# Ulixes-8/UNet-Implementations

Measured on AMD Instinct MI355X. Metric: images/sec (512x512, bs/GPU=8) Our_UNet train step, higher is better.
Workload: dtype f32; 1 GPU; Our_UNet 6-stage 3-class 512x512 bs=8/GPU fp32 train step (fwd + Dice/wCE loss + bwd + SGD-Nesterov), train mode, HIP conv/IN/upsample kernels; global_batch=8, parallelism=dp1, world=1

## Files before the change

include/unet_hip.h:

```cpp
#ifndef UNET_HIP_H_
#define UNET_HIP_H_

#include <stddef.h>
#include <stdint.h>

#ifdef __cplusplus
extern "C" {
#endif

#define UNET_ABI_VERSION 11

#define UNET_OK 0
#define UNET_E_INVALID (-1)
#define UNET_E_LAUNCH (-2)
#define UNET_E_WORKSPACE (-3)

typedef void* unet_stream_t;

const char* unet_last_error(void);
int unet_abi_version(void);
int unet_device_count(void);

int unet_debug_set_chunk_limit(int64_t bytes);

// ... 179 lines not shown
int unet_augment_u8(const uint8_t* image, const uint8_t* mask, uint8_t* image_out,
                    uint8_t* mask_out, const float* params, const uint32_t* rng, int N, int H,
                    int W, unet_stream_t stream);

int unet_preprocess_u8(const uint8_t* image_hwc, const uint8_t* mask, float* out_nhwc,
                       int64_t* target, int N, int H, int W, const float* mean3, const float* std3,
                       unet_stream_t stream);


int unet_sgd_nesterov_step(float* params, const float* grads, float* momentum, int64_t n,
                           float lr, float mu, float weight_decay, int first_step,
                           float grad_scale, unet_stream_t stream);

int unet_sgd_nesterov_step_dev(float* params, const float* grads, float* momentum, int64_t n,
                               const float* hyper, int first_step, unet_stream_t stream);

typedef struct unet_act_src {
  const float* x;
  int C;
  const float* alpha;
  const float* beta;
} unet_act_src;

size_t unet_conv_in_fwd_workspace_bytes(int N, int H, int W, int Cout, int stride);
int unet_conv_in_fwd(const unet_act_src* s0, const unet_act_src* s1, float slope, const float* w,
                     const float* bias, int ksize, int stride, float* y, void* workspace,
                     size_t workspace_bytes, int* stats_px_out, int N, int H, int W, int Cout,
                     unet_stream_t stream);
int unet_conv_in_fwd_bf16x3(const unet_act_src* s0, const unet_act_src* s1, float slope,
                            const float* w, const uint16_t* w3, const float* bias, int ksize,
// ... 292 lines not shown
```

unet-implementations_amd/_lib.py:

```python
import ctypes
import os
import subprocess

_HERE = os.path.dirname(os.path.abspath(__file__))
LIB_PATH = os.environ.get("UNET_HIP_LIB") or os.path.join(_HERE, "libunet_hip.so")
CSRC = os.path.join(_HERE, "csrc")

ABI_VERSION = 11

_c = ctypes
_p = _c.c_void_p
_i = _c.c_int
_f = _c.c_float
_sz = _c.c_size_t
_i64 = _c.c_int64



class ActSrc(ctypes.Structure):
    _fields_ = [("x", _p), ("C", _i), ("alpha", _p), ("beta", _p)]


_ps = _c.POINTER(ActSrc)

# ... 56 lines not shown
    "unet_wgrad_defer_flush": (_i, [_p]),
    "unet_wgrad_defer_end": (_i, [_p]),
    "unet_dice_wce_loss_grad": (_i, [_p, _p, _p, _sz, _p, _p, _i, _i, _i, _i, _p]),
    "unet_argmax_dice_counts": (_i, [_p, _p, _p, _p, _i, _i, _i, _i, _p]),
    "unet_eval_confusion": (_i, [_p, _p, _p, _p, _i, _i, _i, _i, _p]),
    "unet_eval_maps": (_i, [_p, _p, _p, _p, _p, _i, _i, _i, _p]),
    "unet_augment_params_per_sample": (_i, []),
    "unet_augment_u8": (_i, [_p, _p, _p, _p, _p, _p, _i, _i, _i, _p]),
    "unet_gradcam_workspace_bytes": (_sz, [_i, _i, _i]),
    "unet_gradcam_weights": (_i, [_p, _i, _p, _p, _sz, _i, _i, _i, _p]),
    "unet_gradcam_map": (_i, [_ps, _i, _f, _p, _p, _p, _sz, _i, _i, _p]),
    "unet_gradcam_heatmap": (_i, [_p, _p, _sz, _p, _i, _i, _i, _i, _i, _p]),
    "unet_preprocess_u8": (_i, [_p, _p, _p, _p, _i, _i, _i, _c.POINTER(_f), _c.POINTER(_f), _p]),
    "unet_sgd_nesterov_step": (_i, [_p, _p, _p, _i64, _f, _f, _f, _i, _f, _p]),
    "unet_sgd_nesterov_step_dev": (_i, [_p, _p, _p, _i64, _p, _i, _p]),
    "unet_conv_in_fwd_workspace_bytes": (_sz, [_i, _i, _i, _i, _i]),
    "unet_conv_in_fwd": (_i, [_ps, _ps, _f, _p, _p, _i, _i, _p, _p, _sz, _c.POINTER(_i), _i, _i, _i,
                              _i, _p]),
    "unet_conv_in_fwd_bf16x3": (_i, [_ps, _ps, _f, _p, _p, _p, _i, _i, _p, _p, _sz, _c.POINTER(_i), _i,
                                     _i, _i, _i, _p]),
    "unet_conv_up_in_fwd_supported": (_i, [_i, _i, _i, _i, _i, _i]),
    "unet_conv_up_in_fwd": (_i, [_ps, _ps, _f, _p, _p, _p, _p, _sz, _c.POINTER(_i), _i, _i, _i, _i,
                                 _p]),
    "unet_conv_in_stats_finalize": (_i, [_p, _p, _sz, _i, _p, _p, _f, _p, _p, _p, _p, _p, _i, _i, _i,
                                         _p]),
    "unet_stem_u8_fwd": (_i, [_p, _c.POINTER(_f), _c.POINTER(_f), _p, _p, _p, _p, _sz,
                              _c.POINTER(_i), _i, _i, _i, _i, _p]),
    "unet_stem_u8_bwd_weight": (_i, [_p, _c.POINTER(_f), _c.POINTER(_f), _p, _p, _p, _sz, _i, _i,
                                     _i, _i, _p]),
    "unet_conv_in_bwd_weight": (_i, [_ps, _f, _p, _p, _i, _i, _i, _i, _p, _sz, _i, _i, _i, _i, _p]),
# ... 144 lines not shown
```

unet-implementations_amd/csrc/conv_wino.hip:

```cpp
#include "conv_params.h"
#include "lds_asm.h"
#include <utility>

namespace unet_conv {
namespace {

typedef int i32x4v __attribute__((ext_vector_type(4)));
template <int I> using wn_ic = std::integral_constant<int, I>;
template <int B, int... I, typename F>
__device__ __forceinline__ void wn_for_impl(std::integer_sequence<int, I...>, F&& f) {
  (f(wn_ic<B + I>{}), ...);
}
template <int B, int E, typename F>
__device__ __forceinline__ void wn_for(F&& f) {
  wn_for_impl<B>(std::make_integer_sequence<int, E - B>{}, f);
}

constexpr int WN_TH = 8, WN_TW = 32;
constexpr int WN_PW = WN_TW + 2, WN_PH = WN_TH + 2;
constexpr int WN_PPIX = WN_PH * WN_PW;
constexpr int WN_BN = 64;
constexpr int WN_KC = 8;
constexpr int WN_RP = 360;
constexpr int WN_BUF = 16 * 64 * WN_KC;
constexpr size_t WN_LDS = (size_t)(4 * WN_BUF + 2 * WN_KC * WN_RP) * sizeof(float);

__host__ __device__ __forceinline__ int wn_swz(int row, int k) {
  return 2 * ((k >> 1) ^ ((row >> 2) & 3)) + (k & 1);
}

struct WinoParams {
  IgemmParams g;
  const float* wu;
};

template <bool ACT, bool STATS, bool BSTATS, bool UP = false>
__global__ __launch_bounds__(512, 2) void conv_wino_kernel(const WinoParams wp) {
  const IgemmParams& p = wp.g;
  extern __shared__ __attribute__((aligned(16))) float smem[];
// ... 403 lines not shown

__device__ __forceinline__ void wino_pack_items(const float* __restrict__ w,
                                                float* __restrict__ uf, float* __restrict__ ud,
                                                int Cout, int Cin, int dir, long long block) {
  float* dst = dir == 0 ? uf : ud;
  if (!dst) return;
  const int Nn = dir == 0 ? Cout : Cin, Kt = dir == 0 ? Cin : Cout;
  const int kchunks = Kt / WN_KC;
  const long long items = (long long)Nn * kchunks;
  const long long idx = block * 256 + threadIdx.x;
  if (idx >= items) return;
  const int nl = (int)(idx & 63);
  const long long rest = idx >> 6;
  const int kc = (int)(rest % kchunks), tn = (int)(rest / kchunks);
  const int nn = tn * WN_BN + nl;
  float u[16][8];
#pragma unroll
  for (int k = 0; k < 8; ++k) {
    const int kk = kc * WN_KC + k;
    const int co = dir == 0 ? nn : kk, ci = dir == 0 ? kk : nn;
    const float* g = w + ((size_t)co * Cin + ci) * 9;
    float t4[4][3];
#pragma unroll
    for (int v = 0; v < 3; ++v) {
      const float g0 = dir == 0 ? g[0 + v] : g[6 + 2 - v];
      const float g1 = dir == 0 ? g[3 + v] : g[3 + 2 - v];
      const float g2 = dir == 0 ? g[6 + v] : g[0 + 2 - v];
      t4[0][v] = g0;
      t4[1][v] = 0.5f * (g0 + g1 + g2);
      t4[2][v] = 0.5f * (g0 - g1 + g2);
      t4[3][v] = g2;
    }
#pragma unroll
    for (int a = 0; a < 4; ++a) {
      u[4 * a + 0][k] = t4[a][0];
      u[4 * a + 1][k] = 0.5f * (t4[a][0] + t4[a][1] + t4[a][2]);
      u[4 * a + 2][k] = 0.5f * (t4[a][0] - t4[a][1] + t4[a][2]);
      u[4 * a + 3][k] = t4[a][2];
    }
  }
  const bool s1 = (nl >> 2) & 1, s2 = (nl >> 3) & 1;
  float* blk = dst + ((size_t)tn * kchunks + kc) * WN_BUF + nl * 8;
#pragma unroll
  for (int x = 0; x < 16; ++x) {
    f32x2v p0 = {u[x][0], u[x][1]}, p1 = {u[x][2], u[x][3]}, p2 = {u[x][4], u[x][5]},
           p3 = {u[x][6], u[x][7]};
    const f32x2v q0 = s1 ? p1 : p0, q1 = s1 ? p0 : p1, q2 = s1 ? p3 : p2, q3 = s1 ? p2 : p3;
    p0 = s2 ? q2 : q0; p1 = s2 ? q3 : q1; p2 = s2 ? q0 : q2; p3 = s2 ? q1 : q3;
    *reinterpret_cast<f32x4*>(blk + x * 512) = f32x4{p0[0], p0[1], p1[0], p1[1]};
    *reinterpret_cast<f32x4*>(blk + x * 512 + 4) = f32x4{p2[0], p2[1], p3[0], p3[1]};
  }
}

__global__ __launch_bounds__(256) void wino_pack_kernel(const float* __restrict__ w,
                                                        float* __restrict__ uf,
                                                        float* __restrict__ ud, int Cout, int Cin) {
  wino_pack_items(w, uf, ud, Cout, Cin, blockIdx.y, blockIdx.x);
}
__global__ __launch_bounds__(256) void wino_pack_batched_kernel(
    const unet_wino_pack_entry* __restrict__ tab, int n) {
  int k = 0;
  for (int q = 1; q < n; ++q)
    if (tab[q].block_begin <= (int)blockIdx.x) k = q;
  const unet_wino_pack_entry e = tab[k];
  wino_pack_items(e.w, e.uf, e.ud, e.Cout, e.Cin, blockIdx.y, (long long)blockIdx.x - e.block_begin);
}
// ... 153 lines not shown
```

unet-implementations_amd/csrc/misc.hip:

```cpp
#include "conv_params.h"

#include <cxxabi.h>
#include <stdlib.h>
#include <string.h>

#include <mutex>
#include <string>
#include <vector>

static thread_local char g_err[512] = "";

void unet_set_error(const char* fmt, ...) {
  va_list ap;
  va_start(ap, fmt);
  vsnprintf(g_err, sizeof(g_err), fmt, ap);
  va_end(ap);
}

extern "C" const char* unet_last_error(void) { return g_err; }

namespace unet_conv {
long long& chunk_limit_bytes() {
  static long long lim = (1LL << 31) - 1;
  return lim;
// ... 513 lines not shown
    float acc = 0.f;
    for (int Y = ylo; Y <= yhi; ++Y) {
      const float cy = bil_coef(Y, sy, h, iy);
      if (cy == 0.f) continue;
      float row = 0.f;
      for (int X = xlo; X <= xhi; ++X) {
        const float cx = bil_coef(X, sx, w, ix);
        if (cx != 0.f) row += cx * g[(size_t)Y * W + X];
      }
      acc += cy * row;
    }
    gx[i] = acc;
  }
}

__global__ __launch_bounds__(256) void sgd_nesterov_kernel(float* __restrict__ p,
                                                           const float* __restrict__ g,
                                                           float* __restrict__ buf, long long n,
                                                           float lr, float mu, float wd,
                                                           int first_step, float gscale,
                                                           const float* __restrict__ hyper) {
  if (hyper) { lr = hyper[0]; mu = hyper[1]; wd = hyper[2]; gscale = hyper[3]; }
  const long long stride = (long long)gridDim.x * 256;
  const long long n4 = n >> 2;
  for (long long i = (long long)blockIdx.x * 256 + threadIdx.x; i < n4; i += stride) {
    f32x4 pv = *reinterpret_cast<f32x4*>(p + i * 4);
    f32x4 gv = *reinterpret_cast<const f32x4*>(g + i * 4) * gscale + pv * wd;
    f32x4 bv;
    if (first_step) bv = gv;
    else bv = *reinterpret_cast<f32x4*>(buf + i * 4) * mu + gv;
    *reinterpret_cast<f32x4*>(buf + i * 4) = bv;
    gv += bv * mu;
    pv -= gv * lr;
    *reinterpret_cast<f32x4*>(p + i * 4) = pv;
  }
  if (blockIdx.x == 0 && threadIdx.x < (n & 3)) {
    const long long i = (n4 << 2) + threadIdx.x;
    float pv = p[i];
    float gv = g[i] * gscale + pv * wd;
    float bv = first_step ? gv : buf[i] * mu + gv;
    buf[i] = bv;
    gv += bv * mu;
    p[i] = pv - gv * lr;
  }
}

unsigned stream_grid(long long items) {
  long long b = ceil_div64(items, 256);
  if (b > 256 * 16) b = 256 * 16;
  if (b < 1) b = 1;
  return (unsigned)b;
}

}

extern "C" int unet_nchw_to_nhwc(const float* x, float* y, int N, int C, int H, int W,
                                 unet_stream_t stream) {
  UNET_REQUIRE(x && y && N > 0 && C > 0 && H > 0 && W > 0, "nchw_to_nhwc: bad argument");
// ... 149 lines not shown

extern "C" int unet_sgd_nesterov_step_dev(float* params, const float* grads, float* momentum,
                                          int64_t n, const float* hyper, int first_step,
                                          unet_stream_t stream) {
  UNET_REQUIRE(params && grads && momentum && hyper && n > 0, "sgd_nesterov_step_dev: bad argument");
  UNET_REQUIRE(((uintptr_t)params % 16 == 0) && ((uintptr_t)grads % 16 == 0) &&
                   ((uintptr_t)momentum % 16 == 0),
               "sgd_nesterov_step_dev: arenas must be 16-byte aligned");
  hipLaunchKernelGGL(sgd_nesterov_kernel, dim3(stream_grid((n + 3) / 4)), dim3(256), 0,
                     (hipStream_t)stream, params, grads, momentum, (long long)n, 0.f, 0.f, 0.f,
                     first_step, 1.f, hyper);
  UNET_CHECK_LAUNCH("sgd_nesterov(dev)");
  return UNET_OK;
}

extern "C" int unet_transpose2d(const float* src, float* dst, int R, int C, unet_stream_t stream) {
  UNET_REQUIRE(src && dst && R > 0 && C > 0, "transpose2d: bad argument");
  hipLaunchKernelGGL(transpose2d_kernel, dim3(ceil_div(C, 32), ceil_div(R, 32)), dim3(256), 0,
                     (hipStream_t)stream, src, dst, R, C);
  UNET_CHECK_LAUNCH("transpose2d");
  return UNET_OK;
}

extern "C" int unet_preprocess_u8(const uint8_t* image_hwc, const uint8_t* mask, float* out_nhwc,
                                  int64_t* target, int N, int H, int W, const float* mean3,
                                  const float* std3, unet_stream_t stream) {
  UNET_REQUIRE(image_hwc && out_nhwc && mean3 && std3 && N > 0 && H > 0 && W > 0 &&
                   (mask == nullptr || target != nullptr),
               "preprocess_u8: bad argument");
  const long long pixels = (long long)N * H * W;
// ... 30 lines not shown
```

unet-implementations_amd/ddp.py:

```python
import torch
import torch.distributed as dist


class GradBucketAllReduce:

    def __init__(self, model, optimizer=None, process_group=None, bucket_bytes=16 << 20,
                 average=True, always_reduce=False):
        if not dist.is_initialized():
            raise RuntimeError("torch.distributed must be initialised (backend nccl or gloo)")
        self.model = model
        self.group = process_group
        self.world = dist.get_world_size(process_group)
        self.bucket_elems = max(1, bucket_bytes // 4)
        self._works = []
        self._hi = None
        self._prefix = 0
        self.sent_ranges = []
        self.always_reduce = always_reduce
        model.grad_ready_hook = self._on_ready
        if optimizer is not None:
            optimizer.grad_scale = 1.0 / self.world if average else 1.0

    def _on_ready(self, lo):
        garena = getattr(self.model, "_grad_arena", None)
# ... 41 lines not shown

    def finish(self):
        self.check_gradients_alias_arena()
        if self._hi is not None and self._hi > 0 and (self.world > 1 or self.always_reduce):
            _, garena = self.model.flat_parameters()
            self._launch(garena, self._prefix, self._hi)
        for w in self._works:
            w.wait()
        self._works = []
        self._hi = None


def broadcast_parameters(model, src=0, process_group=None):
    arena, _ = model.flat_parameters()
    dist.broadcast(arena, src=src, group=process_group)
```

unet-implementations_amd/ops.py:

```python
import ctypes
import functools
import struct
import threading

import torch

from ._lib import ActSrc, BwdStats, check, lib


_raw_stream = getattr(torch._C, "_cuda_getCurrentRawStream", None)
_raw_device = getattr(torch._C, "_cuda_getDevice", None)


def _stream():
    if _raw_stream is not None and _raw_device is not None:
        return _raw_stream(_raw_device())
    return torch.cuda.current_stream().cuda_stream


class KernelTimer:

    def __init__(self, only=None):
        self.only = only
        self.records = []
# ... 182 lines not shown
        wd = _f32((9, Cin, Cout), w_oihw)
    check(lib().unet_pack_conv3x3_weights(_ptr(w_oihw), _ptr(wf), _ptr(wd), Cout, Cin, _stream()))
    return wf, wd


def pack_conv3x3_weights_bf16x3(w_oihw, want_wd=True, want_wf=True):
    Cout, Cin, kh, kw = w_oihw.shape
    assert kh == 3 and kw == 3
    wf3 = torch.empty((3, 9, Cout, Cin), dtype=torch.bfloat16, device=w_oihw.device) \
        if want_wf else None
    wd3 = torch.empty((3, 9, Cin, Cout), dtype=torch.bfloat16, device=w_oihw.device) \
        if want_wd else None
    check(lib().unet_pack_conv3x3_weights_bf16x3(_ptr(w_oihw), _ptr(wf3), _ptr(wd3), Cout, Cin,
                                                 _stream()))
    return wf3, wd3


class PackTable:

    def __init__(self, weights, planes, wino=None):
        self.wf, self.wd, self.wf3, self.wd3 = [], [], [], []
        self.src_ptrs = [w.data_ptr() for w in weights]
        self.planes = planes
        self.wino = tuple(wino) if wino is not None else tuple((False, False) for _ in weights)
        self.uf, self.ud, self._wino_jobs = [], [], []
        for w, (ff, fd) in zip(weights, self.wino):
            cout, cin = w.shape[0], w.shape[1]
            uf = _f32((16 * cout * cin,), w) if ff else None
            ud = _f32((16 * cout * cin,), w) if fd else None
            self.uf.append(uf)
# ... 19 lines not shown
            wf = _f32((9, cout, cin), w)
            wd = _f32((9, cin, cout), w)
            wf3 = wd3 = None
            if planes and cin != 3:
                npl = 1 if planes == 1 and planes is not True else 3
                wf3 = torch.empty((npl, 9, cout, cin), dtype=torch.bfloat16, device=w.device)
                wd3 = torch.empty((npl, 9, cin, cout), dtype=torch.bfloat16, device=w.device)
            self.wf.append(wf); self.wd.append(wd); self.wf3.append(wf3); self.wd3.append(wd3)
            raw += struct.pack("<5Q4i", w.data_ptr(), wf.data_ptr(), wd.data_ptr(),
                               0 if wf3 is None else wf3.data_ptr(),
                               0 if wd3 is None else wd3.data_ptr(), cout, cin, tiles,
                               1 if (wf3 is not None and wf3.shape[0] == 1) else 0)
            tiles += (cout // 32) * ((cin + 31) // 32)
        self.n, self.tiles = len(weights), tiles
        self.table = torch.frombuffer(bytearray(raw), dtype=torch.uint8).to(weights[0].device)

    def matches(self, weights, planes, wino=None):
        wino = tuple(wino) if wino is not None else tuple((False, False) for _ in weights)
        return planes == self.planes and len(weights) == self.n and wino == self.wino and \
            all(w.data_ptr() == p for w, p in zip(weights, self.src_ptrs))

    def run(self):
        check(lib().unet_pack_conv3x3_weights_batched(self.table.data_ptr(), self.n, self.tiles,
                                                      _stream()))
        if self._wino_table is not None:
            check(lib().unet_pack_wino_weights_batched(self._wino_table.data_ptr(),
                                                       len(self._wino_jobs), self._wino_blocks,
                                                       _stream()))


_PREC = {False: 0, True: 1, 0: 0, 1: 1, 3: 3, "fp32": 0, "bf16": 1, "bf16x3": 3}
_SUFFIX = {0: "", 1: "_bf16", 3: "_bf16x3"}


def _prec(bf16):
    try:
        return _PREC[bf16]
    except (KeyError, TypeError):
        raise ValueError("precision must be 'fp32', 'bf16' or 'bf16x3'") from None


@functools.lru_cache(maxsize=None)
def _sel_conv3x3_fwd(pr, C0):
# ... 897 lines not shown
    n = params.numel()
    t0 = _begin()
    check(lib().unet_sgd_nesterov_step(_ptr(params), _ptr(grads), _ptr(momentum), n, lr, mu,
                                       weight_decay, 1 if first_step else 0, grad_scale,
                                       _stream()))
    if t0 is not None:
        _timer.end("sgd_nesterov", 0.0, 1, t0, nbytes=4.0 * (5 if not first_step else 4) * n)


def sgd_nesterov_step_dev(params, grads, momentum, hyper, first_step):
    n = params.numel()
    check(lib().unet_sgd_nesterov_step_dev(_ptr(params), _ptr(grads), _ptr(momentum), n,
                                           _ptr(hyper), 1 if first_step else 0, _stream()))


def recon3x3_fwd(x, slope, w, b):
    x, rx = _act(x)
    N, H, W, C = x.shape
    K = w.shape[0]
    out = _f32((N, K, H, W), x.x)
    t0 = _begin()
    check(lib().unet_recon3x3_fwd(rx, 1 if _is_b16(x.x) else 0, slope, _ptr(w), _ptr(b),
                                  _ptr(out), N, H, W, K, _stream()))
    if t0 is not None:
        _timer.end("recon_fwd", 2.0 * N * H * W * K * C * 9, 1, t0,
                   nbytes=x.x.element_size() * x.x.numel() + 4.0 * out.numel())
    return out


_recon_ws = {}
# ... 218 lines not shown
```

unet-implementations_amd/optim.py:

```python
import torch

from . import ops


class FusedSGD(torch.optim.Optimizer):
    def __init__(self, params, lr=1e-3, momentum=0.0, dampening=0.0, weight_decay=0.0,
                 nesterov=False, model=None):
        if dampening != 0.0:
            raise NotImplementedError("FusedSGD implements dampening == 0 (the reference setting)")
        if nesterov and momentum <= 0:
            raise ValueError("Nesterov momentum requires a momentum")
        if not nesterov:
            raise NotImplementedError("FusedSGD implements the Nesterov form used by the reference")
        defaults = dict(lr=lr, momentum=momentum, dampening=dampening, weight_decay=weight_decay,
                        nesterov=nesterov)
        super().__init__(params, defaults)
        self._model = model
        self._flat_buf = None
        self._steps = 0
        self.grad_scale = 1.0
        self._hyper = None
        self._hyper_host = None

    def use_device_hyper(self, on=True):
# ... 53 lines not shown
                self._flat_buf[off:off + p.numel()].view_as(p).copy_(st["momentum_buffer"])
                fresh = False
            st["momentum_buffer"] = self._flat_buf[off:off + p.numel()].view_as(p)
        return fresh

    def _snapshot(self):
        self.adopt_flat_momentum()
        return self._flat_buf.detach().clone(), self._steps

    def _restore(self, snap):
        self._flat_buf.copy_(snap[0])
        self._steps = snap[1]

    def _advanced(self):
        self._steps += 1

    @torch.no_grad()
    def step(self, closure=None):
        loss = None
        if closure is not None:
            with torch.enable_grad():
                loss = closure()
        flat = self._flat_ready()
        if not flat and self.grad_scale != 1.0 and self._model is not None:
            m = self._model
            _, garena = m.flat_parameters()
            for (name, p), off in zip(m.named_parameters(), m._offsets):
                if p.grad is not None and p.grad.data_ptr() != garena.data_ptr() + 4 * off:
                    raise RuntimeError(f"{name}.grad does not alias the gradient arena the "
                                       "all-reduce operates on")
        if flat:
            g = self.param_groups[0]
            arena, garena = self._model.flat_parameters()
            first = bool(self.adopt_flat_momentum())
            if self._hyper is not None:
                self.sync_device_hyper()
                ops.sgd_nesterov_step_dev(arena, garena, self._flat_buf, self._hyper, first)
            else:
                ops.sgd_nesterov_step(arena, garena, self._flat_buf, g["lr"], g["momentum"],
                                      g["weight_decay"], first, self.grad_scale)
        else:
            if self._hyper is not None:
                raise RuntimeError("device-side hyper-parameters need the flat-arena step (every "
                                   "parameter and gradient a view of the UNet arenas)")
            for g in self.param_groups:
                for p in g["params"]:
                    if p.grad is None:
                        continue
                    st = self.state[p]
                    first = "momentum_buffer" not in st or st["momentum_buffer"] is None
                    if first:
                        st["momentum_buffer"] = torch.zeros_like(p)
                    if p.data_ptr() % 16 or p.grad.data_ptr() % 16 or not p.is_contiguous() \
                            or not p.grad.is_contiguous():
                        raise RuntimeError("FusedSGD needs contiguous, 16-byte aligned tensors")
                    ops.sgd_nesterov_step(p.data.view(-1), p.grad.view(-1),
# ... 129 lines not shown
    @torch.no_grad()
    def step(self, closure=None):
        loss = None
        if closure is not None:
            with torch.enable_grad():
                loss = closure()
        flat = self._flat_ready()
        if not flat and self.grad_scale != 1.0 and self._model is not None:
            m = self._model
            _, garena = m.flat_parameters()
            for (name, p), off in zip(m.named_parameters(), m._offsets):
                if p.grad is not None and p.grad.data_ptr() != garena.data_ptr() + 4 * off:
                    raise RuntimeError(f"{name}.grad does not alias the gradient arena the "
                                       "all-reduce operates on")
        self.sync_device_hyper()
        if flat:
            arena, garena = self._model.flat_parameters()
            self.adopt_flat_moments()
            ops.adam_step(arena, garena, self._flat_m, self._flat_v, self._hyper, True)
        else:
            first = True
            for p in self.param_groups[0]["params"]:
                if p.grad is None:
                    continue
                if p.grad.is_sparse:
                    raise RuntimeError("FusedAdam does not support sparse gradients")
                st = self.state[p]
                if st.get("exp_avg") is None:
                    st["exp_avg"] = torch.zeros_like(p, memory_format=torch.preserve_format)
                    st["exp_avg_sq"] = torch.zeros_like(p, memory_format=torch.preserve_format)
# ... 11 lines not shown
```

unet-implementations_amd/train.py:

```python
import torch

from . import ops
from .losses import SimpleLoss
from .optim import FusedAdam, FusedSGD
from .unet import UNet


def create_model(device="cuda"):
    model = UNet(in_channels=3, num_classes=3, n_stages=6,
                 features_per_stage=[32, 64, 128, 256, 512, 512], kernel_sizes=[[3, 3]] * 6,
                 strides=[[1, 1], [2, 2], [2, 2], [2, 2], [2, 2], [2, 2]],
                 n_conv_per_stage=[2] * 6, n_conv_per_stage_decoder=[2] * 5, conv_bias=True,
                 norm_op=torch.nn.InstanceNorm2d, norm_op_kwargs={"eps": 1e-5, "affine": True},
                 dropout_op=None, nonlin=torch.nn.LeakyReLU, nonlin_kwargs={"inplace": True},
                 encoder_dropout_rates=[0.0, 0.0, 0.1, 0.2, 0.3, 0.3],
                 decoder_dropout_rates=[0.3, 0.2, 0.2, 0.1, 0.0])
    return model.to(device)


def create_optimizer(model, lr=0.005, weight_decay=1e-4, momentum=0.99):
    return FusedSGD(model.parameters(), lr=lr, weight_decay=weight_decay, momentum=momentum,
                    nesterov=True, model=model)


# ... 52 lines not shown
        with torch.cuda.stream(side):
            for _ in range(max(1, warmup)):
                train_step(model, optimizer, loss_function, self.images, self.masks,
                           grad_sync=finish, input_layout=input_layout)
        cur.wait_stream(side)
        self.graph = torch.cuda.CUDAGraph()
        mode = "thread_local" if grad_sync is not None else "global"
        if grad_sync is not None:
            torch.cuda.synchronize()
        with torch.cuda.graph(self.graph, capture_error_mode=mode):
            self.loss = train_step(model, optimizer, loss_function, self.images, self.masks,
                                   grad_sync=finish, input_layout=input_layout)
        with torch.no_grad():
            arena.copy_(keep_arena)
            optimizer._restore(keep_opt)

    def __call__(self, images, masks):
        if images.shape != self.images.shape or masks.shape != self.masks.shape:
            raise ValueError("GraphedTrainStep was captured for batches of shape "
                             f"{tuple(self.images.shape)} / {tuple(self.masks.shape)}")
        if images.dtype != self.images.dtype or masks.dtype != self.masks.dtype:
            raise ValueError("GraphedTrainStep was captured for batches of dtype "
                             f"{self.images.dtype} / {self.masks.dtype}")
        if images.data_ptr() != self.images.data_ptr():
            self.images.copy_(images, non_blocking=True)
        if masks.data_ptr() != self.masks.data_ptr():
            self.masks.copy_(masks, non_blocking=True)
        self.optimizer.sync_device_hyper()
        self.graph.replay()
        self.optimizer._advanced()
        return self.loss


@torch.no_grad()
def validate(model, val_loader, loss_function, device, ignore_label=255, input_layout=None):
    model.eval()
    val_loss = torch.zeros((), device=device)
    dice_sum = torch.zeros(3, device=device, dtype=torch.float64)
    n = 0
    for batch in val_loader:
        images = batch["image"].to(device, non_blocking=True)
        masks = batch["mask"].to(device, non_blocking=True)
        outputs = model(images) if input_layout is None else \
            model(images, input_layout=input_layout)
# ... 91 lines not shown
```

unet-implementations_amd/unet.py:

```python
from typing import Dict, List, Optional, Tuple, Type, Union

import torch
import torch.nn as nn

from . import ops


class SpatialDropout2d(nn.Module):

    def __init__(self, drop_prob):
        super().__init__()
        self.drop_prob = drop_prob

    def extra_repr(self):
        return f"drop_prob={self.drop_prob}"

    def draw_mask(self, n, channels, device):
        mask = torch.empty(n, channels, 1, 1, device=device).bernoulli_(1 - self.drop_prob)
        return mask.div_(1 - self.drop_prob).view(n, channels)

    def forward(self, x):
        if not self.training or self.drop_prob == 0:
            return x
        return x * self.draw_mask(x.size(0), x.size(1), x.device).view(x.size(0), x.size(1), 1, 1)
# ... 266 lines not shown
                        n_convs=n_conv_per_stage_decoder[lvl],
                        spatial_dropout_rate=decoder_dropout_rates[s], **common))
        self._build_head(features_per_stage[0], num_classes)
        self.initialize_weights()
        self._plan = None
        self._arena = None
        self._grad_arena = None
        self._offsets = None
        self.dropout_mask_override = None
        self.grad_ready_hook = None
        self.matmul_precision = "fp32"
        self.fused_pipeline = True
        self.winograd = True
        self.fullres_folds = True
        self.wgrad32_folds = True
        self.input_mean, self.input_std = ops.IMAGENET_MEAN, ops.IMAGENET_STD

    def _build_bottleneck(self, common):
        """Hook for variants that add modules between encoder and decoder (CLIPUNet)."""

    def _build_head(self, in_features, out_channels):
        self.segmentation_output = nn.Conv2d(in_features, out_channels, kernel_size=1, stride=1,
                                             padding=0, bias=True)

    def _head_module(self):
        return self.segmentation_output

    def _check_head(self):
        head = self.segmentation_output
        if _as_int(head.kernel_size) != 1 or head.in_channels != 32 or head.out_channels != 3:
# ... 264 lines not shown
        convs = [l.conv.weight for l in layers if l.ksize == 3]
        wino = None
        if mode == "fp32" and model.fused_pipeline and model.winograd:
            wino = []
            for l in layers:
                if l.ksize != 3:
                    continue
                co, ci = l.conv.weight.shape[0], l.conv.weight.shape[1]
                s1 = l.stride == 1 and min(co, ci) >= 64
                wino.append((s1 and co % 64 == 0 and ci % 8 == 0,
                             s1 and ci % 64 == 0 and co % 8 == 0))
        table = model.__dict__.get("_pack_table")
        planes = 3 if mode == "bf16x3" else (1 if (mode == "bf16" and model.fused_pipeline) else False)
        if table is None or not table.matches(convs, planes, wino):
            table = model.__dict__["_pack_table"] = ops.PackTable(convs, planes, wino)
        table.run()
        self.table = table
        self.row = {id(w): k for k, w in enumerate(convs)}

    def weight_forms(self, l, s0, s1, up=False):
        w = l.conv.weight
        if l.ksize == 1:
            w2d = w.detach().view(w.shape[0], w.shape[1])
            return (w2d, None, None), \
                (ops.transpose2d(w2d) if self.need_grad else None, None, None, None)
        t, k = self.table, self.row[id(w)]
        wu = ud = ud1 = None
        if self.fused and self.mode == "fp32":
            n, h, w_ = (s1 if up else s0).shape[:3]
            c0, c1, cout = s0.shape[3], 0 if s1 is None else s1.shape[3], w.shape[0]
            if t.uf[k] is not None and s0.alpha is not None and \
                    (s1 is None or s1.alpha is not None) and \
                    (ops.conv_up_wino_supported if up else ops.conv_wino_supported)(
                        n, h, w_, c0, c1, cout):
                wu = t.uf[k]
            if t.ud[k] is not None:
                if up:
                    if self.need_grad and ops.conv_wino_supported(n, h, w_, cout, 0, c1):
                        ud1 = t.ud[k]
                elif c1 == 0 and ops.conv_wino_supported(n, h, w_, cout, 0, c0):
                    ud = t.ud[k]
        return (t.wf[k], t.wf3[k], wu), (t.wd[k], t.wd3[k], ud, ud1)

    def run_layer(self, l, x0, x1, place):
        (w, w3, _), bwd_forms = self.weight_forms(l, x0, x1)
        if l.ksize == 1:
            y = ops.conv1x1_fwd(x0, x1, w, l.conv.bias.detach())
        else:
            y = ops.conv3x3_fwd(x0, x1, w, l.conv.bias.detach(), l.stride, bf16=self.mode, wf3=w3)
        st = ops.instnorm_stats(y, l.norm.weight.detach(), l.norm.bias.detach(), l.norm.eps)
        m = self.mask_of[id(l)]
        a = ops.instnorm_lrelu_drop_fwd(y, st[2], st[3], m, l.slope)
        if self.need_grad:
            self.saved.append(_Rec(l, x0, x1, y, st, m, bwd_forms, place, a=a))
        return a

# ... 106 lines not shown
        if l.ksize == 1:
            if want_dw:
                dw2d = dw.view(dw.shape[0], dw.shape[1])
                ops.conv1x1_bwd_weight(x0, dy, dw2d, 0)
                if x1 is not None:
                    ops.conv1x1_bwd_weight(x1, dy, dw2d, x0.shape[3])
            dx0 = ops.conv1x1_bwd_data(dy, rec.wd, 0, x0.shape[3]) if need_dx else None
            return dx0, None
        if want_dw:
            ops.conv3x3_bwd_weight(x0, dy, dw, 0, l.stride, bf16=self.mode)
            if x1 is not None:
                ops.conv3x3_bwd_weight(x1, dy, dw, x0.shape[3], l.stride, bf16=self.mode)
        dx0 = dx1 = None
        N, H, W, C0 = x0.shape
        if need_dx:
            dx0 = ops.conv3x3_bwd_data(dy, rec.wd, 0, C0, H, W, l.stride, out=dx0_acc,
                                       accumulate=dx0_acc is not None, bf16=self.mode,
                                       wd3=rec.wd3, nxt=nxt, ud=rec.ud)
        if x1 is not None and need_dx1:
            dx1 = ops.conv3x3_bwd_data(dy, rec.wd, C0, x1.shape[3], H, W, l.stride,
                                       bf16=self.mode, wd3=rec.wd3)
        return dx0, dx1


class _UNetFunction(torch.autograd.Function):
    @staticmethod
    def forward(ctx, model, x, extra, *params):
        c32_mode = "always" if ops.c32_winograd_override() == "always" else bool(model.winograd)
        with ops.c32_winograd_scope(c32_mode):
            logits = _UNetFunction._forward(ctx, model, x, extra, params)
# ... 168 lines not shown
```

Before: 480.2 images/s.

## Fuse weight-form repacking into the SGD Nesterov optimizer step

The SGD Nesterov kernel now also writes the packed conv weight forms (the transposed forward/backward layouts and the Winograd-transformed forms) from the freshly updated parameters, held in an LDS tile. This lets the next forward pass skip the separate pack pass and its extra read of the weight arena. The model tracks which forms each layer actually needs so the kernel writes only those, with a partial skip for split-input layers. In exchange it adds freshness and validity bookkeeping across the optimizer, DDP broadcast and graph replay, plus a scattered, transposing write pattern in the optimizer kernel.

```diff
diff --git a/include/unet_hip.h b/include/unet_hip.h
--- a/include/unet_hip.h
+++ b/include/unet_hip.h
@@ -217,6 +217,25 @@
 
 int unet_sgd_nesterov_step_dev(float* params, const float* grads, float* momentum, int64_t n,
                                const float* hyper, int first_step, unet_stream_t stream);
+
+typedef struct unet_sgd_forms_row {
+  int64_t begin;
+  int64_t count;
+  float* wf;
+  float* wd;
+  float* uf;
+  float* ud;
+  int Cout, Cin;
+  int block_begin;
+  int mask;
+  int ud_ci_begin;
+  int reserved;
+} unet_sgd_forms_row;
+int unet_sgd_nesterov_step_forms(float* params, const float* grads, float* momentum, int64_t n,
+                                 const unet_sgd_forms_row* table_device, int rows,
+                                 int total_blocks, float lr, float mu, float weight_decay,
+                                 int first_step, float grad_scale, const float* hyper,
+                                 unet_stream_t stream);
 
 typedef struct unet_act_src {
   const float* x;
diff --git a/unet-implementations_amd/_lib.py b/unet-implementations_amd/_lib.py
--- a/unet-implementations_amd/_lib.py
+++ b/unet-implementations_amd/_lib.py
@@ -94,6 +94,8 @@
     "unet_preprocess_u8": (_i, [_p, _p, _p, _p, _i, _i, _i, _c.POINTER(_f), _c.POINTER(_f), _p]),
     "unet_sgd_nesterov_step": (_i, [_p, _p, _p, _i64, _f, _f, _f, _i, _f, _p]),
     "unet_sgd_nesterov_step_dev": (_i, [_p, _p, _p, _i64, _p, _i, _p]),
+    "unet_sgd_nesterov_step_forms": (_i, [_p, _p, _p, _i64, _p, _i, _i, _f, _f, _f, _i, _f, _p,
+                                          _p]),
     "unet_conv_in_fwd_workspace_bytes": (_sz, [_i, _i, _i, _i, _i]),
     "unet_conv_in_fwd": (_i, [_ps, _ps, _f, _p, _p, _i, _i, _p, _p, _sz, _c.POINTER(_i), _i, _i, _i,
                               _i, _p]),
diff --git a/unet-implementations_amd/csrc/conv_wino.hip b/unet-implementations_amd/csrc/conv_wino.hip
--- a/unet-implementations_amd/csrc/conv_wino.hip
+++ b/unet-implementations_amd/csrc/conv_wino.hip
@@ -1,5 +1,6 @@
 #include "conv_params.h"
 #include "lds_asm.h"
+#include "wino_pack.h"
 #include <utility>
 
 namespace unet_conv {
@@ -23,6 +24,7 @@
 constexpr int WN_KC = 8;
 constexpr int WN_RP = 360;
 constexpr int WN_BUF = 16 * 64 * WN_KC;
+static_assert(WN_BN == WNP_BN && WN_KC == WNP_KC && WN_BUF == WNP_BUF, "wino_pack.h writes this image");
 constexpr size_t WN_LDS = (size_t)(4 * WN_BUF + 2 * WN_KC * WN_RP) * sizeof(float);
 
 __host__ __device__ __forceinline__ int wn_swz(int row, int k) {
@@ -456,42 +458,12 @@
   const long long rest = idx >> 6;
   const int kc = (int)(rest % kchunks), tn = (int)(rest / kchunks);
   const int nn = tn * WN_BN + nl;
-  float u[16][8];
-#pragma unroll
-  for (int k = 0; k < 8; ++k) {
+  const bool rot = dir != 0;
+  wino_pack_item(dst + ((size_t)tn * kchunks + kc) * WN_BUF, nl, rot, [&](int k, int t) {
     const int kk = kc * WN_KC + k;
-    const int co = dir == 0 ? nn : kk, ci = dir == 0 ? kk : nn;
-    const float* g = w + ((size_t)co * Cin + ci) * 9;
-    float t4[4][3];
-#pragma unroll
-    for (int v = 0; v < 3; ++v) {
-      const float g0 = dir == 0 ? g[0 + v] : g[6 + 2 - v];
-      const float g1 = dir == 0 ? g[3 + v] : g[3 + 2 - v];
-      const float g2 = dir == 0 ? g[6 + v] : g[0 + 2 - v];
-      t4[0][v] = g0;
-      t4[1][v] = 0.5f * (g0 + g1 + g2);
-      t4[2][v] = 0.5f * (g0 - g1 + g2);
-      t4[3][v] = g2;
-    }
-#pragma unroll
-    for (int a = 0; a < 4; ++a) {
-      u[4 * a + 0][k] = t4[a][0];
-      u[4 * a + 1][k] = 0.5f * (t4[a][0] + t4[a][1] + t4[a][2]);
-      u[4 * a + 2][k] = 0.5f * (t4[a][0] - t4[a][1] + t4[a][2]);
-      u[4 * a + 3][k] = t4[a][2];
-    }
-  }
-  const bool s1 = (nl >> 2) & 1, s2 = (nl >> 3) & 1;
-  float* blk = dst + ((size_t)tn * kchunks + kc) * WN_BUF + nl * 8;
-#pragma unroll
-  for (int x = 0; x < 16; ++x) {
-    f32x2v p0 = {u[x][0], u[x][1]}, p1 = {u[x][2], u[x][3]}, p2 = {u[x][4], u[x][5]},
-           p3 = {u[x][6], u[x][7]};
-    const f32x2v q0 = s1 ? p1 : p0, q1 = s1 ? p0 : p1, q2 = s1 ? p3 : p2, q3 = s1 ? p2 : p3;
-    p0 = s2 ? q2 : q0; p1 = s2 ? q3 : q1; p2 = s2 ? q0 : q2; p3 = s2 ? q1 : q3;
-    *reinterpret_cast<f32x4*>(blk + x * 512) = f32x4{p0[0], p0[1], p1[0], p1[1]};
-    *reinterpret_cast<f32x4*>(blk + x * 512 + 4) = f32x4{p2[0], p2[1], p3[0], p3[1]};
-  }
+    const int co = rot ? kk : nn, ci = rot ? nn : kk;
+    return w[((size_t)co * Cin + ci) * 9 + t];
+  });
 }
 
 __global__ __launch_bounds__(256) void wino_pack_kernel(const float* __restrict__ w,
diff --git a/unet-implementations_amd/csrc/misc.hip b/unet-implementations_amd/csrc/misc.hip
--- a/unet-implementations_amd/csrc/misc.hip
+++ b/unet-implementations_amd/csrc/misc.hip
@@ -1,4 +1,5 @@
 #include "conv_params.h"
+#include "wino_pack.h"
 
 #include <cxxabi.h>
 #include <stdlib.h>
@@ -551,6 +552,43 @@
   }
 }
 
+template <bool TAIL>
+__device__ __forceinline__ void sgd_nesterov_update(float& p, float g, float& b, bool first_step,
+                                                    float lr, float mu, float wd, float gscale) {
+#pragma clang fp contract(off)
+  const float t = g * gscale;
+  float gv;
+  if (TAIL) {
+    const float pw = p * wd;
+    gv = pw + t;
+  } else {
+    gv = __builtin_fmaf(p, wd, t);
+  }
+  b = first_step ? gv : __builtin_fmaf(b, mu, gv);
+  gv = __builtin_fmaf(b, mu, gv);
+  p = __builtin_fmaf(-lr, gv, p);
+}
+
+__device__ __forceinline__ f32x4 sgd_nesterov_update4(float* __restrict__ p,
+                                                      const float* __restrict__ g,
+                                                      float* __restrict__ buf, long long i,
+                                                      bool first_step, float lr, float mu,
+                                                      float wd, float gscale) {
+  f32x4 pv = *reinterpret_cast<f32x4*>(p + i);
+  const f32x4 gv = *reinterpret_cast<const f32x4*>(g + i);
+  f32x4 bv = {0.f, 0.f, 0.f, 0.f};
+  if (!first_step) bv = *reinterpret_cast<f32x4*>(buf + i);
+#pragma unroll
+  for (int k = 0; k < 4; ++k) {
+    float pk = pv[k], bk = bv[k];
+    sgd_nesterov_update<false>(pk, gv[k], bk, first_step, lr, mu, wd, gscale);
+    pv[k] = pk; bv[k] = bk;
+  }
+  *reinterpret_cast<f32x4*>(buf + i) = bv;
+  *reinterpret_cast<f32x4*>(p + i) = pv;
+  return pv;
+}
+
 __global__ __launch_bounds__(256) void sgd_nesterov_kernel(float* __restrict__ p,
                                                            const float* __restrict__ g,
                                                            float* __restrict__ buf, long long n,
@@ -560,25 +598,100 @@
   if (hyper) { lr = hyper[0]; mu = hyper[1]; wd = hyper[2]; gscale = hyper[3]; }
   const long long stride = (long long)gridDim.x * 256;
   const long long n4 = n >> 2;
-  for (long long i = (long long)blockIdx.x * 256 + threadIdx.x; i < n4; i += stride) {
-    f32x4 pv = *reinterpret_cast<f32x4*>(p + i * 4);
-    f32x4 gv = *reinterpret_cast<const f32x4*>(g + i * 4) * gscale + pv * wd;
-    f32x4 bv;
-    if (first_step) bv = gv;
-    else bv = *reinterpret_cast<f32x4*>(buf + i * 4) * mu + gv;
-    *reinterpret_cast<f32x4*>(buf + i * 4) = bv;
-    gv += bv * mu;
-    pv -= gv * lr;
-    *reinterpret_cast<f32x4*>(p + i * 4) = pv;
-  }
+  for (long long i = (long long)blockIdx.x * 256 + threadIdx.x; i < n4; i += stride)
+    sgd_nesterov_update4(p, g, buf, i * 4, first_step != 0, lr, mu, wd, gscale);
   if (blockIdx.x == 0 && threadIdx.x < (n & 3)) {
     const long long i = (n4 << 2) + threadIdx.x;
-    float pv = p[i];
-    float gv = g[i] * gscale + pv * wd;
-    float bv = first_step ? gv : buf[i] * mu + gv;
+    float pv = p[i], bv = first_step ? 0.f : buf[i];
+    sgd_nesterov_update<true>(pv, g[i], bv, first_step != 0, lr, mu, wd, gscale);
     buf[i] = bv;
-    gv += bv * mu;
-    p[i] = pv - gv * lr;
+    p[i] = pv;
+  }
+}
+
+constexpr int SGDF_RANGE = 4096;
+
+__global__ __launch_bounds__(256) void sgd_nesterov_forms_kernel(
+    float* __restrict__ p, const float* __restrict__ g, float* __restrict__ buf, long long n,
+    const unet_sgd_forms_row* __restrict__ tab, int rows, float lr, float mu, float wd,
+    int first_step, float gscale, const float* __restrict__ hyper) {
+  __shared__ float tile[32][289];
+  if (hyper) { lr = hyper[0]; mu = hyper[1]; wd = hyper[2]; gscale = hyper[3]; }
+  const bool first = first_step != 0;
+  int lo = 0, hi = rows - 1;
+  while (lo < hi) {
+    const int mid = (lo + hi + 1) >> 1;
+    if (tab[mid].block_begin <= (int)blockIdx.x) lo = mid; else hi = mid - 1;
+  }
+  const unet_sgd_forms_row e = tab[lo];
+  const int id = blockIdx.x - e.block_begin;
+  const long long nv = n & ~3LL;
+  if (e.count > 0) {
+    const long long b = e.begin + (long long)id * SGDF_RANGE;
+    long long end = b + SGDF_RANGE;
+    if (end > e.begin + e.count) end = e.begin + e.count;
+    if (end > n) end = n;
+    const long long vend = end < nv ? end : nv;
+    for (long long i = b + 4 * (long long)threadIdx.x; i < vend; i += 1024)
+      sgd_nesterov_update4(p, g, buf, i, first, lr, mu, wd, gscale);
+    for (long long i = (b > nv ? b : nv) + threadIdx.x; i < end; i += 256) {
+      float pv = p[i], bv = first ? 0.f : buf[i];
+      sgd_nesterov_update<true>(pv, g[i], bv, first, lr, mu, wd, gscale);
+      buf[i] = bv;
+      p[i] = pv;
+    }
+    return;
+  }
+  const int tiles_ci = (e.Cin + 31) / 32;
+  const int co0 = (id / tiles_ci) * 32, ci0 = (id % tiles_ci) * 32;
+  if (co0 >= e.Cout || e.begin + (long long)9 * e.Cin * e.Cout > nv) return;
+  const int nci = min(32, e.Cin - ci0), run = nci * 9;
+  const long long pitch = (long long)e.Cin * 9;
+  const long long base = e.begin + ((long long)co0 * e.Cin + ci0) * 9;
+  if ((e.Cin & 3) == 0) {
+    const int r4 = run >> 2;
+    for (int idx = threadIdx.x; idx < 32 * r4; idx += 256) {
+      const int co = idx / r4, j = idx - co * r4;
+      const f32x4 pv = sgd_nesterov_update4(p, g, buf, base + co * pitch + 4 * j, first, lr, mu,
+                                            wd, gscale);
+      float* t = &tile[co][4 * j];
+      t[0] = pv[0]; t[1] = pv[1]; t[2] = pv[2]; t[3] = pv[3];
+    }
+  } else {
+    for (int idx = threadIdx.x; idx < 32 * run; idx += 256) {
+      const int co = idx / run, jj = idx - co * run;
+      const long long i = base + co * pitch + jj;
+      float pv = p[i], bv = first ? 0.f : buf[i];
+      sgd_nesterov_update<false>(pv, g[i], bv, first, lr, mu, wd, gscale);
+      buf[i] = bv;
+      p[i] = pv;
+      tile[co][jj] = pv;
+    }
+  }
+  __syncthreads();
+  if ((e.mask & 1) && e.wf)
+    for (int idx = threadIdx.x; idx < 9 * 32 * nci; idx += 256) {
+      const int tp = idx / (32 * nci), rem = idx - tp * 32 * nci;
+      const int co = rem / nci, ci = rem - co * nci;
+      e.wf[((size_t)tp * e.Cout + co0 + co) * e.Cin + ci0 + ci] = tile[co][ci * 9 + tp];
+    }
+  if ((e.mask & 2) && e.wd)
+    for (int idx = threadIdx.x; idx < 9 * nci * 32; idx += 256) {
+      const int tp = idx / (nci * 32), rem = idx - tp * nci * 32;
+      const int ci = rem >> 5, co = rem & 31;
+      e.wd[((size_t)tp * e.Cin + ci0 + ci) * e.Cout + co0 + co] = tile[co][ci * 9 + tp];
+    }
+  const int it = threadIdx.x & 127, col = it & 31, kcl = it >> 5;
+  if (threadIdx.x < 128) {
+    if ((e.mask & 4) && e.uf && kcl < (nci >> 3)) {
+      const int nn = co0 + col, kchunks = e.Cin / WNP_KC, kc = (ci0 >> 3) + kcl;
+      wino_pack_item(e.uf + ((size_t)(nn >> 6) * kchunks + kc) * WNP_BUF, nn & 63, false,
+                     [&](int k, int t) { return tile[col][(kcl * 8 + k) * 9 + t]; });
+    }
+  } else if ((e.mask & 8) && e.ud && ci0 >= e.ud_ci_begin && col < nci) {
+    const int nn = ci0 + col, kchunks = e.Cout / WNP_KC, kc = (co0 >> 3) + kcl;
+    wino_pack_item(e.ud + ((size_t)(nn >> 6) * kchunks + kc) * WNP_BUF, nn & 63, true,
+                   [&](int k, int t) { return tile[kcl * 8 + k][col * 9 + t]; });
   }
 }
 
@@ -758,6 +871,24 @@
   return UNET_OK;
 }
 
+extern "C" int unet_sgd_nesterov_step_forms(float* params, const float* grads, float* momentum,
+                                            int64_t n, const unet_sgd_forms_row* table_device,
+                                            int rows, int total_blocks, float lr, float mu,
+                                            float weight_decay, int first_step, float grad_scale,
+                                            const float* hyper, unet_stream_t stream) {
+  UNET_REQUIRE(params && grads && momentum && table_device && n > 0 && rows > 0 &&
+                   total_blocks > 0,
+               "sgd_nesterov_step_forms: bad argument");
+  UNET_REQUIRE(((uintptr_t)params % 16 == 0) && ((uintptr_t)grads % 16 == 0) &&
+                   ((uintptr_t)momentum % 16 == 0),
+               "sgd_nesterov_step_forms: arenas must be 16-byte aligned");
+  hipLaunchKernelGGL(sgd_nesterov_forms_kernel, dim3((unsigned)total_blocks), dim3(256), 0,
+                     (hipStream_t)stream, params, grads, momentum, (long long)n, table_device,
+                     rows, lr, mu, weight_decay, first_step, grad_scale, hyper);
+  UNET_CHECK_LAUNCH("sgd_nesterov_forms");
+  return UNET_OK;
+}
+
 extern "C" int unet_transpose2d(const float* src, float* dst, int R, int C, unet_stream_t stream) {
   UNET_REQUIRE(src && dst && R > 0 && C > 0, "transpose2d: bad argument");
   hipLaunchKernelGGL(transpose2d_kernel, dim3(ceil_div(C, 32), ceil_div(R, 32)), dim3(256), 0,
diff --git a/unet-implementations_amd/csrc/wino_pack.h b/unet-implementations_amd/csrc/wino_pack.h
--- /dev/null
+++ b/unet-implementations_amd/csrc/wino_pack.h
@@ -0,0 +1,46 @@
+#pragma once
+#include "common.h"
+
+constexpr int WNP_BN = 64;
+constexpr int WNP_KC = 8;
+constexpr int WNP_BUF = 16 * WNP_BN * WNP_KC;
+
+template <typename Tap>
+__device__ __forceinline__ void wino_pack_item(float* __restrict__ blk, int nl, bool rot,
+                                               Tap&& tap) {
+#pragma clang fp contract(off)
+  const bool s1 = (nl >> 2) & 1, s2 = (nl >> 3) & 1;
+  float* row = blk + nl * 8;
+#pragma unroll
+  for (int h = 0; h < 2; ++h) {
+    float u[16][4];
+#pragma unroll
+    for (int k = 0; k < 4; ++k) {
+      float g[9];
+#pragma unroll
+      for (int t = 0; t < 9; ++t) g[t] = tap(4 * h + k, rot ? 8 - t : t);
+      float t4[4][3];
+#pragma unroll
+      for (int v = 0; v < 3; ++v) {
+        const float g0 = g[0 + v], g1 = g[3 + v], g2 = g[6 + v];
+        t4[0][v] = g0;
+        t4[1][v] = 0.5f * (g0 + g1 + g2);
+        t4[2][v] = 0.5f * (g0 - g1 + g2);
+        t4[3][v] = g2;
+      }
+#pragma unroll
+      for (int a = 0; a < 4; ++a) {
+        u[4 * a + 0][k] = t4[a][0];
+        u[4 * a + 1][k] = 0.5f * (t4[a][0] + t4[a][1] + t4[a][2]);
+        u[4 * a + 2][k] = 0.5f * (t4[a][0] - t4[a][1] + t4[a][2]);
+        u[4 * a + 3][k] = t4[a][2];
+      }
+    }
+    float* slot = row + 4 * (h ^ (int)s2);
+#pragma unroll
+    for (int x = 0; x < 16; ++x)
+      *reinterpret_cast<f32x4*>(slot + x * 512) =
+          s1 ? f32x4{u[x][2], u[x][3], u[x][0], u[x][1]}
+             : f32x4{u[x][0], u[x][1], u[x][2], u[x][3]};
+  }
+}
diff --git a/unet-implementations_amd/ddp.py b/unet-implementations_amd/ddp.py
--- a/unet-implementations_amd/ddp.py
+++ b/unet-implementations_amd/ddp.py
@@ -79,3 +79,4 @@
 def broadcast_parameters(model, src=0, process_group=None):
     arena, _ = model.flat_parameters()
     dist.broadcast(arena, src=src, group=process_group)
+    model.__dict__["_arena_writes"] = model.__dict__.get("_arena_writes", 0) + 1
diff --git a/unet-implementations_amd/ops.py b/unet-implementations_amd/ops.py
--- a/unet-implementations_amd/ops.py
+++ b/unet-implementations_amd/ops.py
@@ -220,6 +220,36 @@
     check(lib().unet_pack_conv3x3_weights_bf16x3(_ptr(w_oihw), _ptr(wf3), _ptr(wd3), Cout, Cin,
                                                  _stream()))
     return wf3, wd3
+
+
+FORM_WF, FORM_WD, FORM_UF, FORM_UD, FORM_UD_SKIP = 1, 2, 4, 8, 16
+SGD_FORMS_RANGE = 4096
+
+
+def sgd_forms_layout(n, convs):
+    nv = n - n % 4
+    order = sorted(range(len(convs)), key=lambda k: convs[k][0])
+    tile_rows, ranges, blocks, pos = [None] * len(convs), [], 0, 0
+    for k in order:
+        begin, cout, cin = convs[k]
+        end = begin + 9 * cout * cin
+        if begin % 4 or cout % 32 or cin <= 0 or begin < pos or end > nv:
+            raise ValueError("sgd_forms_layout: a 3x3 weight needs a 16-byte aligned offset, Cout a "
+                             "multiple of 32, and must lie inside the arena's float4 body without "
+                             "overlapping its neighbour")
+        if begin > pos:
+            ranges.append((pos, begin - pos))
+        pos = end
+    if n > pos:
+        ranges.append((pos, n - pos))
+    for k, (begin, cout, cin) in enumerate(convs):
+        tile_rows[k] = (begin, cout, cin, blocks)
+        blocks += (cout // 32) * ((cin + 31) // 32)
+    range_rows = []
+    for begin, count in ranges:
+        range_rows.append((begin, count, blocks))
+        blocks += (count + SGD_FORMS_RANGE - 1) // SGD_FORMS_RANGE
+    return tile_rows, range_rows, blocks
 
 
 class PackTable:
@@ -269,6 +299,101 @@
             tiles += (cout // 32) * ((cin + 31) // 32)
         self.n, self.tiles = len(weights), tiles
         self.table = torch.frombuffer(bytearray(raw), dtype=torch.uint8).to(weights[0].device)
+        self.weights = list(weights)
+        self.read = None
+        self.prev_read = None
+        self.valid = [0] * self.n
+        self._fresh = None
+        self._sgd_tables = {}
+        self.ud_begin = [0] * self.n
+
+    def _all_forms(self, k):
+        return FORM_WF | FORM_WD | (FORM_UF if self.uf[k] is not None else 0) | \
+            ((FORM_UD | FORM_UD_SKIP) if self.ud[k] is not None else 0)
+
+    def stamp(self, model):
+        arena = getattr(model, "_arena", None)
+        if arena is None:
+            return None
+        return (arena.data_ptr(), arena._version, sum(w._version for w in self.weights),
+                model.__dict__.get("_arena_writes", 0))
+
+    def fresh_for(self, model):
+        return self._fresh is not None and self._fresh == self.stamp(model)
+
+    def begin_walk(self, model):
+        if not (getattr(model, "sgd_emits_forms", False) and self.fresh_for(model)):
+            self.run()
+        self.prev_read, self.read = self.read, [0] * self.n
+
+    def need(self, k, form):
+        if self.read is not None:
+            self.read[k] |= form
+        have = self.valid[k]
+        if have & form or (form == FORM_UD_SKIP and have & FORM_UD):
+            return
+        w = self.weights[k]
+        cout, cin = w.shape[0], w.shape[1]
+        if form in (FORM_WF, FORM_WD):
+            check(lib().unet_pack_conv3x3_weights(
+                _ptr(w), _ptr(self.wf[k] if form == FORM_WF else None),
+                _ptr(self.wd[k] if form == FORM_WD else None), cout, cin, _stream()))
+        else:
+            if form != FORM_UF:
+                form = FORM_UD | FORM_UD_SKIP
+            check(lib().unet_pack_wino_weights(
+                _ptr(w), _ptr(self.uf[k] if form == FORM_UF else None),
+                _ptr(self.ud[k] if form != FORM_UF else None), cout, cin, _stream()))
+        self.valid[k] = have | form
+
+    def in_arena(self, arena):
+        base, n = arena.data_ptr(), arena.numel()
+        return all(w.data_ptr() == p and p >= base and (p - base) % 16 == 0 and
+                   (p - base) // 4 + w.numel() <= n for w, p in zip(self.weights, self.src_ptrs))
+
+    def sgd_table(self, arena, masks, ud_begin):
+        key = (arena.data_ptr(), arena.numel(), tuple(masks), tuple(ud_begin))
+        hit = self._sgd_tables.get(key)
+        if hit is not None:
+            return hit
+        base = arena.data_ptr()
+        convs = []
+        for w in self.weights:
+            off = w.data_ptr() - base
+            if off < 0 or off % 4 or off // 4 + w.numel() > arena.numel():
+                raise ValueError("sgd_table: a 3x3 weight is not a view of the arena")
+            convs.append((off // 4, w.shape[0], w.shape[1]))
+        tile_rows, range_rows, blocks = sgd_forms_layout(arena.numel(), convs)
+        raw = b""
+        for k, (begin, cout, cin, b0) in enumerate(tile_rows):
+            m = masks[k]
+            bits = (m & (FORM_WF | FORM_WD | FORM_UF)) | \
+                (FORM_UD if m & (FORM_UD | FORM_UD_SKIP) else 0)
+            if (self.uf[k] is not None and (cout % 64 or cin % 8)) or \
+                    (self.ud[k] is not None and (cin % 64 or cout % 8)) or ud_begin[k] % 32:
+                raise ValueError("sgd_table: a Winograd form needs 64 | columns and 8 | channels")
+            ptrs = [0 if t is None else t.data_ptr()
+                    for t in (self.wf[k], self.wd[k], self.uf[k], self.ud[k])]
+            raw += struct.pack("<2q4Q6i", begin, 0, *ptrs, cout, cin, b0, bits,
+                               0 if m & FORM_UD else ud_begin[k], 0)
+        for begin, count, b0 in range_rows:
+            raw += struct.pack("<2q4Q6i", begin, count, 0, 0, 0, 0, 0, 0, b0, 0, 0, 0)
+        dev = torch.frombuffer(bytearray(raw), dtype=torch.uint8).to(arena.device)
+        hit = self._sgd_tables[key] = (dev, len(tile_rows) + len(range_rows), blocks)
+        return hit
+
+    def forms_bytes(self, masks):
+        total = 0
+        for k, m in enumerate(masks):
+            e = self.weights[k].numel()
+            total += 4 * e * (bool(m & FORM_WF) + bool(m & FORM_WD)) + \
+                4 * (16 * e // 9) * bool(m & FORM_UF)
+            if m & FORM_UD:
+                total += 4 * (16 * e // 9)
+            elif m & FORM_UD_SKIP:
+                cin = self.weights[k].shape[1]
+                total += 4 * (16 * e // 9) * (cin - self.ud_begin[k]) // cin
+        return total
 
     def matches(self, weights, planes, wino=None):
         wino = tuple(wino) if wino is not None else tuple((False, False) for _ in weights)
@@ -282,6 +407,8 @@
             check(lib().unet_pack_wino_weights_batched(self._wino_table.data_ptr(),
                                                        len(self._wino_jobs), self._wino_blocks,
                                                        _stream()))
+        self.valid = [self._all_forms(k) for k in range(self.n)]
+        self._fresh = None
 
 
 _PREC = {False: 0, True: 1, 0: 0, 1: 1, 3: 3, "fp32": 0, "bf16": 1, "bf16x3": 3}
@@ -1209,6 +1336,19 @@
                                            _ptr(hyper), 1 if first_step else 0, _stream()))
 
 
+def sgd_nesterov_step_forms(params, grads, momentum, table, masks, lr, mu, weight_decay,
+                            first_step, grad_scale=1.0, hyper=None):
+    n = params.numel()
+    dev, rows, blocks = table.sgd_table(params, masks, table.ud_begin)
+    t0 = _begin() if hyper is None else None
+    check(lib().unet_sgd_nesterov_step_forms(
+        _ptr(params), _ptr(grads), _ptr(momentum), n, dev.data_ptr(), rows, blocks, lr, mu,
+        weight_decay, 1 if first_step else 0, grad_scale, _ptr(hyper), _stream()))
+    if t0 is not None:
+        _timer.end("sgd_nesterov", 0.0, 1, t0,
+                   nbytes=4.0 * (5 if not first_step else 4) * n + table.forms_bytes(masks))
+
+
 def recon3x3_fwd(x, slope, w, b):
     x, rx = _act(x)
     N, H, W, C = x.shape
diff --git a/unet-implementations_amd/optim.py b/unet-implementations_amd/optim.py
--- a/unet-implementations_amd/optim.py
+++ b/unet-implementations_amd/optim.py
@@ -1,6 +1,11 @@
 import torch
 
 from . import ops
+
+
+def _arena_written(model):
+    if model is not None:
+        model.__dict__["_arena_writes"] = model.__dict__.get("_arena_writes", 0) + 1
 
 
 class FusedSGD(torch.optim.Optimizer):
@@ -91,6 +96,15 @@
 
     def _advanced(self):
         self._steps += 1
+
+    def _forms_table(self):
+        m = self._model
+        table = m.__dict__.get("_pack_table")
+        if not getattr(m, "sgd_emits_forms", False) or table is None or table.planes or \
+                table.read is None or table.read != table.prev_read or \
+                getattr(m, "grad_ready_hook", None) is not None or not table.in_arena(m._arena):
+            return None
+        return table
 
     @torch.no_grad()
     def step(self, closure=None):
@@ -112,11 +126,22 @@
             first = bool(self.adopt_flat_momentum())
             if self._hyper is not None:
                 self.sync_device_hyper()
+            table = self._forms_table()
+            _arena_written(self._model)
+            if table is not None:
+                masks = list(table.read)
+                ops.sgd_nesterov_step_forms(arena, garena, self._flat_buf, table, masks, g["lr"],
+                                            g["momentum"], g["weight_decay"], first,
+                                            self.grad_scale, hyper=self._hyper)
+                table.valid = masks
+                table._fresh = table.stamp(self._model)
+            elif self._hyper is not None:
                 ops.sgd_nesterov_step_dev(arena, garena, self._flat_buf, self._hyper, first)
             else:
                 ops.sgd_nesterov_step(arena, garena, self._flat_buf, g["lr"], g["momentum"],
                                       g["weight_decay"], first, self.grad_scale)
         else:
+            _arena_written(self._model)
             if self._hyper is not None:
                 raise RuntimeError("device-side hyper-parameters need the flat-arena step (every "
                                    "parameter and gradient a view of the UNet arenas)")
@@ -276,6 +301,7 @@
                     raise RuntimeError(f"{name}.grad does not alias the gradient arena the "
                                        "all-reduce operates on")
         self.sync_device_hyper()
+        _arena_written(self._model)
         if flat:
             arena, garena = self._model.flat_parameters()
             self.adopt_flat_moments()
diff --git a/unet-implementations_amd/train.py b/unet-implementations_amd/train.py
--- a/unet-implementations_amd/train.py
+++ b/unet-implementations_amd/train.py
@@ -90,6 +90,9 @@
         with torch.no_grad():
             arena.copy_(keep_arena)
             optimizer._restore(keep_opt)
+        table = model.__dict__.get("_pack_table")
+        self._table = table if table is not None and table._fresh is not None else None
+        self._forms = list(table.valid) if self._table is not None else None
 
     def __call__(self, images, masks):
         if images.shape != self.images.shape or masks.shape != self.masks.shape:
@@ -103,7 +106,16 @@
         if masks.data_ptr() != self.masks.data_ptr():
             self.masks.copy_(masks, non_blocking=True)
         self.optimizer.sync_device_hyper()
+        table = self._table
+        if table is not None:
+            if not table.fresh_for(self.model) or \
+                    any(f & ~v for f, v in zip(self._forms, table.valid)):
+                table.run()
+        self.model.__dict__["_arena_writes"] = self.model.__dict__.get("_arena_writes", 0) + 1
         self.graph.replay()
+        if table is not None:
+            table.valid = list(self._forms)
+            table._fresh = table.stamp(self.model)
         self.optimizer._advanced()
         return self.loss
 
diff --git a/unet-implementations_amd/unet.py b/unet-implementations_amd/unet.py
--- a/unet-implementations_amd/unet.py
+++ b/unet-implementations_amd/unet.py
@@ -304,6 +304,7 @@
         self.winograd = True
         self.fullres_folds = True
         self.wgrad32_folds = True
+        self.sgd_emits_forms = True
         self.input_mean, self.input_std = ops.IMAGENET_MEAN, ops.IMAGENET_STD
 
     def _build_bottleneck(self, common):
@@ -598,7 +599,7 @@
         planes = 3 if mode == "bf16x3" else (1 if (mode == "bf16" and model.fused_pipeline) else False)
         if table is None or not table.matches(convs, planes, wino):
             table = model.__dict__["_pack_table"] = ops.PackTable(convs, planes, wino)
-        table.run()
+        table.begin_walk(model)
         self.table = table
         self.row = {id(w): k for k, w in enumerate(convs)}
 
@@ -624,6 +625,19 @@
                         ud1 = t.ud[k]
                 elif c1 == 0 and ops.conv_wino_supported(n, h, w_, cout, 0, c0):
                     ud = t.ud[k]
+        t.need(k, ops.FORM_UF if wu is not None else ops.FORM_WF)
+        if self.need_grad:
+            if ud is None:
+                t.need(k, ops.FORM_WD)
+            else:
+                t.need(k, ops.FORM_UD)
+            if ud1 is not None:
+                c0 = s0.shape[3]
+                if c0 % 32 == 0 and t.ud_begin[k] in (0, c0):
+                    t.ud_begin[k] = c0
+                    t.need(k, ops.FORM_UD_SKIP)
+                else:
+                    t.need(k, ops.FORM_UD)
         return (t.wf[k], t.wf3[k], wu), (t.wd[k], t.wd3[k], ud, ud1)
 
     def run_layer(self, l, x0, x1, place):
@@ -760,6 +774,8 @@
         dx0 = dx1 = None
         N, H, W, C0 = x0.shape
         if need_dx:
+            if rec.ud is not None and dx0_acc is not None:
+                self.table.need(self.row[id(l.conv.weight)], ops.FORM_WD)
             dx0 = ops.conv3x3_bwd_data(dy, rec.wd, 0, C0, H, W, l.stride, out=dx0_acc,
                                        accumulate=dx0_acc is not None, bf16=self.mode,
                                        wd3=rec.wd3, nxt=nxt, ud=rec.ud)
```

After: 483.7 images/s (median of 6 runs). About the same (+0.7%).
